# Dostenlinus/Aiyagari-HARK

Hardware: AMD Instinct MI355X
Metric: GE solves/sec (Table II sweep); agent-periods/sec; % HBM roofline (higher is better)
Workload: dtype f64

## Files before the change

aiyagari_hark_amd/csrc/egm_common.h:

```cpp
#pragma once

#include "common.h"

namespace aiy {

constexpr int kEgmBlock = 256;
constexpr int kTile = 64;
constexpr int kEgmWaves = kEgmBlock / kWave;
constexpr int kSub = 32;
constexpr int kFlag = 3 * kSub;
constexpr int kSlots = 3 * kSub + 4;
constexpr int kWin = 2 * kWave;

constexpr int kHintBack = 8;


template <bool AGENT>
__device__ __forceinline__ double ld_f64(const double* p) {
  if constexpr (AGENT) return load_f64_agent(p);
  else return *p;
}

__device__ __forceinline__ double uniform_f64(double x) {
  const unsigned long long u = (unsigned long long)__double_as_longlong(x);
// ... 94 lines not shown

__device__ __forceinline__ double interp_row_global(const double* __restrict__ xr, const double* __restrict__ yr,
                                                    int n, double q, int& lb) {
  lb = lower_bound(xr, 0, n, q);
  const int i = lb < 1 ? 1 : lb;
  return lerp_at(xr, yr, i, q, xr[0]);
}

__device__ __forceinline__ double interp_row_global_agent(const double* __restrict__ xr,
                                                          const double* __restrict__ yr, int n, double q, int& lb) {
  int lo = 0, hi = n;
  while (lo < hi) {
    const int mid = lo + ((hi - lo) >> 1);
    if (load_f64_agent(&xr[mid]) < q) lo = mid + 1; else hi = mid;
  }
  lb = lo;
  const int i = lb < 1 ? 1 : lb;
  const double xl = load_f64_agent(&xr[i - 1]), xh = load_f64_agent(&xr[i]);
  const double yl = load_f64_agent(&yr[i - 1]), yh = load_f64_agent(&yr[i]);
  const double alpha = (q - xl) / (xh - xl);
  const double v = (1.0 - alpha) * yl + alpha * yh;
  return (q < load_f64_agent(&xr[0])) ? __builtin_nan("") : v;
}

template <int PK>
__device__ __forceinline__ double marg_u(double c, double gam) {
  if constexpr (PK == 1) return 1.0 / c;
  else if constexpr (PK == 3) return 1.0 / ((c * c) * c);
  else if constexpr (PK == 5) {
    const double c2 = c * c;
    return 1.0 / ((c2 * c2) * c);
  } else return pow(c, -gam);
}
template <int PK>
__device__ __forceinline__ double inv_marg(double E, double gam) {
  if constexpr (PK == 1) return 1.0 / E;
  else if constexpr (PK == 3) return rcbrt(E);
  else if constexpr (PK == 5) {
    if (!(E > 1e-30 && E < 1e30)) return pow(E, -0.2);
    double y = (double)powf((float)E, -0.2f);
#pragma unroll
    for (int it = 0; it < 2; ++it) {
      const double y2 = y * y;
      const double e = 1.0 - E * ((y2 * y2) * y);
      y = y + y * (e * 0.2);
    }
    return y;
  } else return pow(E, -1.0 / gam);
}

}
```

aiyagari_hark_amd/csrc/ge_resident.hip:

```cpp
#include "common.h"
#include "egm_common.h"
#include "ge_search.h"
#include "hist_bicg.h"
#include "hist_cluster.h"
#include "internal.h"

#include <algorithm>
#include <cmath>

namespace aiy {

constexpr int kGeTHMax = 1024;
constexpr int kGeWavesMax = kGeTHMax / kWave;
constexpr int kGeMaxTiles = 16;
constexpr int kGeBufs = 5;
constexpr int kGeAaM = 3;
constexpr int kGeAaHist = kGeAaM + 2;
#ifdef AIY_DIAG_NO_FUSEA
constexpr bool kGeFuseA = false;
#else
constexpr bool kGeFuseA = true;
#endif
#ifndef AIY_FUSEA_KC2
#define AIY_FUSEA_KC2 0
#endif
constexpr bool kGeFuseAKc2 = AIY_FUSEA_KC2 != 0;
template <int NW>
constexpr size_t ge_egm_lds() { return (size_t)NW * (8 * kTile + 4 * kWin) * sizeof(double); }

struct GeCalDev {
  double alpha, delta, disc, r_lo, r_hi;
};

struct GeState;
struct GeRun {
  int n_cal, S, n_a, G, nj, cap, n_work;
  const double* a_grid;
  const double* P;
  const double* lab;
  const double* beta;
  const double* crra;
  const GeCalDev* cal;
  int method;
  double r_tol, egm_tol, hist_tol;
  int max_steps, max_cyc, max_hist;
  int warm_hist, warm_egm, secant, loose, extrap;
  int extrap_period;
  int aa_period;
  double* aah;
  int logsec;
  int pull;
  double loose_hist;
  double* qb;
  int* ainv;
  double* tab;
  double* mass;
  double* pmass;
  double* pg;
  int* lo;
  double* wlo;
  double* slab;
  int* span;
  unsigned* ctr;
  unsigned long long* gran;
  const int* cal_ids;
  GeState* saved;
  const int* resume;
  unsigned* done_ctr;
  int stop_at;
  int* out_done;
  unsigned* err;
  double* out_r;
  double* out_K;
  double* out_Ks;
  int* out_steps;
  int* out_cyc;
  int* out_its;
  int* out_status;
  double* out_prof;
  double* out_evlog;
};
constexpr int kGeProf = 8;
constexpr int kGeEvLog = 32;
constexpr int kGeEvRec = 6;
// ... 8 lines not shown
  long long cyc_sum, its_sum;
  unsigned long long t_egm, t_lot, t_hist, t_k, t0, t_ev0;
  unsigned nc_prev[2];
  unsigned nbc;
};

template <int TH>
__device__ __forceinline__ bool ge_reduce(unsigned long long* gran, int G, int w, unsigned& ne, const double* vals,
                                          int nv, unsigned kmax, double (*s_part)[kGeWavesMax], double* s_res,
                                          int* s_flag, unsigned* err) {
  asm volatile("s_waitcnt vmcnt(0)" ::: "memory");
  return hc_reduce<TH>(gran, G, w, ne, vals, nv, kmax, s_part, s_res, s_flag, err, [] {});
}

template <int SMAX, int NW, typename Sink, typename Begin, typename End>
__device__ __forceinline__ void ge_rows_pass(int S, int n_a, int j0, int j1, const double* __restrict__ a_grid,
                                             const double* __restrict__ src_m, const double* __restrict__ src_c,
                                             double R, const double* s_Wl, int* s_hint, double* lds_win,
                                             Sink&& sink, Begin&& begin, End&& end) {
  const int tid = threadIdx.x, lane = tid & (kWave - 1);
  const int wv = __builtin_amdgcn_readfirstlane(tid / kWave);
  const int n = n_a, n1 = n_a + 1;
  const int ntile = (j1 - j0 + kTile - 1) / kTile;
  double* X = lds_win + (size_t)wv * 4 * kWin;
  double* Y = X + kWin;
  double* XB = X + 2 * kWin;
  double* YB = X + 3 * kWin;
#pragma unroll 1
  for (int tile = wv; tile < ntile; tile += NW) {
    const int jr = j0 + tile * kTile + lane;
    const int j = jr < j1 ? jr : j1 - 1;
    const double a = a_grid[j];
    int* hint = s_hint + tile * SMAX;
    begin(tile, j);
    auto fetch = [&](int r, RowWin& wn) {
      const int rr = r < S ? r : S - 1;
      load_win<true>(src_m + (size_t)rr * n1, src_c + (size_t)rr * n1, n, win_base(hint[rr], n1), lane, wn);
    };
    unsigned redo = 0u;
    auto step_unit = [&](int u, const RowWin& wa, const RowWin& wb) {
      const int ra = 2 * u, rb = 2 * u + 1;
      if (ra >= S) return;
      const bool has_b = rb < S;
      const int rbb = has_b ? rb : ra;
      const bool na = __any(stage_win(wa, n, X, Y, lane));
      const bool nb = __any(stage_win(wb, n, XB, YB, lane));
      __builtin_amdgcn_fence(__ATOMIC_RELEASE, "wavefront");
      __builtin_amdgcn_wave_barrier();
      __builtin_amdgcn_fence(__ATOMIC_ACQUIRE, "wavefront");
      const double qa = R * a + s_Wl[ra];
      const double qb = R * a + s_Wl[rbb];
      int lba, lbb;
      bool oka, okb;
      const double fa = search_win(wa.base, na, n, qa, X, Y, lba, oka);
      const double fb = search_win(wb.base, nb, n, qb, XB, YB, lbb, okb);
      hint[ra] = __builtin_amdgcn_readfirstlane(lba);
      if (has_b) hint[rb] = __builtin_amdgcn_readfirstlane(lbb);
      if (__any(!oka)) redo |= 1u << ra;
      else sink(tile, jr, j, ra, qa, fa);
      if (has_b) {
        if (__any(!okb)) redo |= 1u << rb;
        else sink(tile, jr, j, rb, qb, fb);
      }
    };
    RowWin a0, b0, a1, b1;
    fetch(0, a0);
    fetch(1, b0);
#pragma unroll 1
    for (int u = 0; 2 * u < S; u += 2) {
      fetch(2 * u + 2, a1);
      fetch(2 * u + 3, b1);
      step_unit(u, a0, b0);
      fetch(2 * u + 4, a0);
      fetch(2 * u + 5, b0);
      step_unit(u + 1, a1, b1);
    }
#pragma unroll 1
    while (redo != 0u) {
      const int s = __builtin_ctz(redo);
      redo &= redo - 1u;
      const double q = R * a + s_Wl[s];
      int lb;
      const double f = interp_row_global_agent(src_m + (size_t)s * n1, src_c + (size_t)s * n1, n, q, lb);
      hint[s] = __builtin_amdgcn_readfirstlane(lb);
      sink(tile, jr, j, s, q, f);
    }
    end(tile, j, a);
  }
}

template <int SMAX, int SC, int PK, int NW>
__device__ __forceinline__ double ge_egm_cycle(int S, int n_a, int j0, int j1, const double* __restrict__ a_grid,
                                               const double* src_m, const double* src_c, double* dst_m,
                                               double* dst_c, bool track, double R, double beta, double gam,
                                               const double* s_Wl, const double* s_Pe, int* s_hint,
                                               double* lds_v, double* lds_win, double* ring) {
  const int tid = threadIdx.x, lane = tid & (kWave - 1);
  const int wv = __builtin_amdgcn_readfirstlane(tid / kWave);
  const int n1 = n_a + 1;
  double* Vw = lds_v + (size_t)wv * SMAX * kTile;
  const int ntile = (j1 - j0 + kTile - 1) / kTile;
  double dmax = 0.0;
  if (src_m == nullptr) {
#pragma unroll 1
    for (int tile = wv; tile < ntile; tile += NW) {
      const int jr = j0 + tile * kTile + lane;
      const int j = jr < j1 ? jr : j1 - 1;
      const double a = a_grid[j];
      for (int sp = 0; sp < S; ++sp) {
        const double c = (R * a + s_Wl[sp]) * 1.0;
        Vw[sp * kTile + lane] = R * marg_u<PK>(c, gam);
      }
      for (int s = 0; s < S; ++s) {
        double sum;
        if constexpr (SC > 0) sum = pairwise_dot<SC>(Vw + lane, s_Pe + s * SC);
        else sum = np_pairwise_sum<SMAX>(S, [&](int t) { return Vw[t * kTile + lane] * uniform_f64(s_Pe[s * S + t]); });
        const double c = inv_marg<PK>(beta * sum, gam);
        store_f64_agent(&dst_m[(size_t)s * n1 + j + 1], a + c);
        store_f64_agent(&dst_c[(size_t)s * n1 + j + 1], c);
        if (ring) store_f64_agent(&ring[(size_t)s * n_a + j], c);
        if (j == 0) {
          store_f64_agent(&dst_m[(size_t)s * n1], kBorrowNode);
          store_f64_agent(&dst_c[(size_t)s * n1], kBorrowNode);
        }
      }
    }
    return 0.0;
  }
  constexpr int NP = SC > 0 ? SC : SMAX;
  double pmv[NP], pcv[NP];
  auto begin = [&](int, int j) {
#pragma unroll
    for (int s = 0; s < NP; ++s) {
      pmv[s] = 0.0;
      pcv[s] = 0.0;
      if (track && s < S) {
        pmv[s] = load_f64_agent(&src_m[(size_t)s * n1 + j + 1]);
        pcv[s] = load_f64_agent(&src_c[(size_t)s * n1 + j + 1]);
      }
    }
  };
  auto end = [&](int, int j, double a) {
#pragma unroll
    for (int s = 0; s < NP; ++s) {
      if (s < S) {
        __builtin_amdgcn_sched_barrier(0);
        double sum;
        if constexpr (SC > 0) sum = pairwise_dot<SC>(Vw + lane, s_Pe + s * SC);
        else sum = np_pairwise_sum<SMAX>(S, [&](int t) { return Vw[t * kTile + lane] * uniform_f64(s_Pe[s * S + t]); });
        const double E = beta * sum;
        const double c = inv_marg<PK>(E, gam);
        const double m = a + c;
        store_f64_agent(&dst_m[(size_t)s * n1 + j + 1], m);
        store_f64_agent(&dst_c[(size_t)s * n1 + j + 1], c);
        if (ring) store_f64_agent(&ring[(size_t)s * n_a + j], c);
        if (track) dmax = nan_max(dmax, nan_max(fabs(m - pmv[s]), fabs(c - pcv[s])));
        if (j == 0) {
          store_f64_agent(&dst_m[(size_t)s * n1], kBorrowNode);
          store_f64_agent(&dst_c[(size_t)s * n1], kBorrowNode);
        }
      }
    }
  };
  ge_rows_pass<SMAX, NW>(S, n_a, j0, j1, a_grid, src_m, src_c, R, s_Wl, s_hint, lds_win,
                     [&](int, int, int, int sp, double, double f) {
                       Vw[sp * kTile + lane] = R * marg_u<PK>(f, gam);
                     },
                     begin, end);
  return dmax;
}

constexpr int kGeSmax = 8;
extern __shared__ double ge_dyn[];
__shared__ double ge_s_part[kHcRed][kGeWavesMax];
__shared__ double ge_s_res[kHcRed];
__shared__ int ge_s_flag;
__shared__ double ge_s_Pe[kGeSmax * kGeSmax];
__shared__ double ge_s_Wl[kGeSmax];
__shared__ int ge_s_hint[kGeMaxTiles * kGeSmax];
__shared__ unsigned ge_s_nc;
__shared__ GeState ge_st;

template <int SMAX, int SC, int PK, int NW>
__device__ __forceinline__ double ge_egm_cycle_fn(int S, int n_a, int j0, int j1, const double* a_grid,
                                               const double* src_m, const double* src_c, double* dst_m,
                                               double* dst_c, bool track, double R, double beta, double gam,
                                               double* ring) {
  return ge_egm_cycle<SMAX, SC, PK, NW>(S, n_a, j0, j1, a_grid, src_m, src_c, dst_m, dst_c, track, R, beta, gam,
                                        ge_s_Wl, ge_s_Pe, ge_s_hint, ge_dyn, ge_dyn + (size_t)NW * SMAX * kTile, ring);
}

template <int SMAX, int NW>
__device__ __forceinline__ void ge_lottery_fn(int S, int n_a, int j0, int j1, const double* a_grid, const double* fm,
                                           const double* fc, double R, bool have_prev, int* LO, double* WL,
                                           bool write_through) {
  ge_rows_pass<SMAX, NW>(S, n_a, j0, j1, a_grid, fm, fc, R, ge_s_Wl, ge_s_hint, ge_dyn + (size_t)NW * SMAX * kTile,
                     [&](int, int jr, int, int s, double q, double c) {
                       if (jr >= j1) return;
                       const double ap = q - c;
                       const size_t o = (size_t)s * n_a + jr;
                       int d = -1;
                       if (have_prev) {
                         const int h = LO[o];
                         if (h >= 0 && h < n_a - 1 && a_grid[h] <= ap && ap < a_grid[h + 1]) d = h;
                       }
                       if (d < 0) {
                         int lo = 0, hi = n_a;
                         while (lo < hi) {
                           const int mid = lo + ((hi - lo) >> 1);
                           if (a_grid[mid] <= ap) lo = mid + 1; else hi = mid;
                         }
                         d = lo - 1;
                       }
                       d = d < 0 ? 0 : (d > n_a - 2 ? n_a - 2 : d);
                       double wl = (a_grid[d + 1] - ap) / (a_grid[d + 1] - a_grid[d]);
                       wl = wl < 0.0 ? 0.0 : (wl > 1.0 ? 1.0 : wl);
                       if (write_through) {
                         __hip_atomic_store(to_global(&LO[o]), d, __ATOMIC_RELAXED, __HIP_MEMORY_SCOPE_AGENT);
                         store_f64_agent(&WL[o], wl);
                       } else {
                         LO[o] = d;
                         WL[o] = wl;
                       }
                     },
                     [](int, int) {}, [](int, int, double) {});
}

struct GeCtx {
  double* tab;
  double* X;
  double* PX;
  int* LO;
  double* WL;
  unsigned* ctr;
  unsigned long long* cw;
  unsigned long long* gran;
  const double* a_grid;
  double beta, gam;
  size_t tab_sz;
  int j0, j1, w, G, S, n_a, cal, lc;
  __device__ __forceinline__ double* tabm(int b) const { return tab + (size_t)b * 2 * tab_sz; }
  __device__ __forceinline__ double* tabc(int b) const { return tab + (size_t)b * 2 * tab_sz + tab_sz; }
};

__device__ __forceinline__ GeEvalOpts ge_eval_opts(const GeRun& g) {
  return {g.method, g.loose, g.logsec, g.warm_egm, g.warm_hist, g.secant, g.r_tol, g.egm_tol, g.hist_tol, g.loose_hist};
}

__device__ __forceinline__ bool ge_barrier(const GeCtx& cx, unsigned& nb, unsigned* err) {
  asm volatile("s_waitcnt vmcnt(0)" ::: "memory");
  ++nb;
  return hc_barrier(err, cx.ctr, (unsigned)cx.G * nb, &ge_s_flag);
}

__device__ __forceinline__ bool ge_vote(const GeCtx& cx, unsigned* err, unsigned flag, unsigned& dlt) {
  GeState& st = ge_st;
  const int tid = threadIdx.x;
  if (tid == 0) ++st.nbc;
  asm volatile("s_waitcnt vmcnt(0)" ::: "memory");
  __syncthreads();
  const unsigned k = st.nbc, par = k & 1u;
  if (!hc_barrier_count(err, &cx.cw[par], (unsigned)cx.G * ((k + par) / 2), flag, &ge_s_nc, &ge_s_flag))
    return false;
  if (tid == 0) {
    dlt = ge_s_nc - st.nc_prev[par];
    st.nc_prev[par] = ge_s_nc;
  }
  return true;
}

template <int TH>
__device__ __forceinline__ void ge_secant_tables(const GeCtx& cx, int b_cur, int b_prev, int b_init, double theta) {
  const int tid = threadIdx.x, n1 = cx.n_a + 1;
  for (int s = 0; s < cx.S; ++s) {
    for (int k = cx.j0 + tid; k < cx.j1; k += TH) {
      const size_t o = (size_t)s * n1 + k + 1;
      const double cm = load_f64_agent(&cx.tabm(b_cur)[o]), pm = load_f64_agent(&cx.tabm(b_prev)[o]);
      const double cc = load_f64_agent(&cx.tabc(b_cur)[o]), pc = load_f64_agent(&cx.tabc(b_prev)[o]);
      store_f64_agent(&cx.tabm(b_init)[o], theta == 0.0 ? cm : cm + theta * (cm - pm));
      store_f64_agent(&cx.tabc(b_init)[o], theta == 0.0 ? cc : cc + theta * (cc - pc));
    }
    if (cx.j0 == 0 && tid == 0) {
      store_f64_agent(&cx.tabm(b_init)[(size_t)s * n1], kBorrowNode);
      store_f64_agent(&cx.tabc(b_init)[(size_t)s * n1], kBorrowNode);
    }
  }
}

template <int SMAX, int SC, int NW>
__device__ __forceinline__ double ge_egm_dispatch(const GeCtx& cx, int pk, const double* sm, const double* sc, double* dm,
                                                  double* dc, bool track, double R, double* ring) {
  if (pk == 1)
    return ge_egm_cycle_fn<SMAX, SC, 1, NW>(cx.S, cx.n_a, cx.j0, cx.j1, cx.a_grid, sm, sc, dm, dc, track, R, cx.beta,
                                            cx.gam, ring);
  if (pk == 3)
    return ge_egm_cycle_fn<SMAX, SC, 3, NW>(cx.S, cx.n_a, cx.j0, cx.j1, cx.a_grid, sm, sc, dm, dc, track, R, cx.beta,
                                            cx.gam, ring);
  if (pk == 5)
    return ge_egm_cycle_fn<SMAX, SC, 5, NW>(cx.S, cx.n_a, cx.j0, cx.j1, cx.a_grid, sm, sc, dm, dc, track, R, cx.beta,
                                            cx.gam, ring);
  return ge_egm_cycle_fn<SMAX, SC, 0, NW>(cx.S, cx.n_a, cx.j0, cx.j1, cx.a_grid, sm, sc, dm, dc, track, R, cx.beta,
                                          cx.gam, ring);
}

template <int TH>
__device__ __forceinline__ bool ge_extrapolate(const GeCtx& cx, unsigned& nb, unsigned* err, int b_dst, int b_src,
                                               double dclu, int n) {
  GeState& st = ge_st;
  const int tid = threadIdx.x, n1 = cx.n_a + 1;
  if (tid == 0) {
    st.fext = egm_extrap_factor(dclu, st.dist, st.ev.etol, n, st.lam_prev);
    if (st.fext != 0.0) st.moved = 1;
  }
  __syncthreads();
  const double f = st.fext;
  if (f != 0.0) {
    double* cm = cx.tabm(b_dst);
    double* cc = cx.tabc(b_dst);
    const double* pm = cx.tabm(b_src);
    const double* pc = cx.tabc(b_src);
    for (int s = 0; s < cx.S; ++s)
      for (int k = cx.j0 + tid; k < cx.j1; k += TH) {
        const size_t o = (size_t)s * n1 + k + 1;
        const double x = load_f64_agent(&cm[o]), y = load_f64_agent(&cc[o]);
        store_f64_agent(&cm[o], x + f * (x - load_f64_agent(&pm[o])));
        store_f64_agent(&cc[o], y + f * (y - load_f64_agent(&pc[o])));
      }
    if (!ge_barrier(cx, nb, err)) return false;
  }
  return true;
}

__device__ __forceinline__ double* ge_ring(const GeCtx& cx, const GeRun& g, int c) {
  return g.aah + ((size_t)cx.cal * kGeAaHist + (size_t)(c % kGeAaHist)) * cx.S * cx.n_a;
}

template <int TH>
__device__ __forceinline__ bool ge_anderson(const GeCtx& cx, unsigned& nb, unsigned& ne, const GeRun& g, int n,
                                            int b_dst) {
  static_assert(kGeAaM == 3 && kGeAaHist == 5, "the mixing is written for m = 3");
  const int tid = threadIdx.x, n1 = cx.n_a + 1;
  const double* W0 = ge_ring(cx, g, n - 4);
  const double* W1 = ge_ring(cx, g, n - 3);
  const double* W2 = ge_ring(cx, g, n - 2);
  const double* W3 = ge_ring(cx, g, n - 1);
  const double* W4 = ge_ring(cx, g, n);
  double gp[9];
  for (int q = 0; q < 9; ++q) gp[q] = 0.0;
  for (int s = 0; s < cx.S; ++s)
    for (int k = cx.j0 + tid; k < cx.j1; k += TH) {
      const size_t o = (size_t)s * cx.n_a + k;
      const double w0 = load_f64_agent(W0 + o), w1 = load_f64_agent(W1 + o), w2 = load_f64_agent(W2 + o);
      const double w3 = load_f64_agent(W3 + o), w4 = load_f64_agent(W4 + o);
      aa_gram_add(w0, w1, w2, w3, w4, gp);
    }
  double gs[9], gam[3];
  if (!ge_reduce<TH>(cx.gran, cx.G, cx.w, ne, gp, 6, 0u, ge_s_part, ge_s_res, &ge_s_flag, g.err)) return false;
  for (int q = 0; q < 6; ++q) gs[q] = ge_s_res[q];
  if (!ge_reduce<TH>(cx.gran, cx.G, cx.w, ne, gp + 6, 3, 0u, ge_s_part, ge_s_res, &ge_s_flag, g.err)) return false;
  for (int q = 0; q < 3; ++q) gs[6 + q] = ge_s_res[q];
  if (aa_solve(gs, gam)) {
    double* dm = cx.tabm(b_dst);
    double* dc = cx.tabc(b_dst);
    for (int s = 0; s < cx.S; ++s)
      for (int k = cx.j0 + tid; k < cx.j1; k += TH) {
        const size_t o = (size_t)s * cx.n_a + k;
        const double w1 = load_f64_agent(W1 + o), w2 = load_f64_agent(W2 + o);
        const double w3 = load_f64_agent(W3 + o), w4 = load_f64_agent(W4 + o);
        const double cn = aa_mix(gam, w1, w2, w3, w4);
        store_f64_agent(&dm[(size_t)s * n1 + k + 1], cx.a_grid[k] + cn);
        store_f64_agent(&dc[(size_t)s * n1 + k + 1], cn);
      }
    if (tid == 0) ge_st.moved = 1;
    if (!ge_barrier(cx, nb, g.err)) return false;
  }
  return true;
}

template <int SMAX, int SC, int TH>
__device__ __forceinline__ int ge_household_solve(const GeCtx& cx, unsigned& nb, unsigned& ne, const GeRun& g, int pk,
                                                  double R, const double* init_m, const double* init_c) {
  constexpr int NW = TH / kWave;
  GeState& st = ge_st;
  const int tid = threadIdx.x;
  int final_buf = -1;
  for (int attempt = 0; attempt < 2; ++attempt) {
    if (!ge_barrier(cx, nb, g.err)) return -1;
    const bool aa = g.aa_period > 0 && attempt == 0;
    const bool ext = st.extrap != 0 && attempt == 0 && !aa;
    if (tid == 0) {
      st.lam_prev = -1.0;
      st.moved = 0;
      st.nan_stop = 0;
    }
    int n = 1;
    const int last_allowed = g.max_cyc + 1;
    bool converged = false;
    while (true) {
      const int b_dst = st.buf[n & 1], b_src = st.buf[(n - 1) & 1];
      const double* sm = n == 1 ? init_m : cx.tabm(b_src);
      const double* sc = n == 1 ? init_c : cx.tabc(b_src);
      const bool track = n >= 2;
      const double dl = ge_egm_dispatch<SMAX, SC, NW>(cx, pk, sm, sc, cx.tabm(b_dst), cx.tabc(b_dst), track, R,
                                                      aa ? ge_ring(cx, g, n) : nullptr);
      const int xp = g.extrap_period;
      const bool want_value = ext && n >= xp - 1 && ((n % xp) == xp - 1 || (n % xp) == 0);
      double dclu = 0.0;
      bool go;
      if (want_value) {
        double v[1] = {dl};
        if (!ge_reduce<TH>(cx.gran, cx.G, cx.w, ne, v, 1, 1u, ge_s_part, ge_s_res, &ge_s_flag, g.err)) return -1;
        dclu = ge_s_res[0];
        go = dclu > st.ev.etol;
        if (tid == 0) st.nan_stop = dclu != dclu;
      } else {
        const double dw = wave_nan_max(dl);
        if ((tid & (kWave - 1)) == 0) ge_s_part[0][tid / kWave] = dw;
        __syncthreads();
        unsigned flag = 0u, dlt = 0u;
        if (tid == 0) {
          double d = ge_s_part[0][0];
          for (int q = 1; q < TH / kWave; ++q) d = nan_max(d, ge_s_part[0][q]);
          flag = (d > st.ev.etol ? 1u : 0u) | (d != d ? (1u << 16) : 0u);
        }
        if (!ge_vote(cx, g.err, flag, dlt)) return -1;
        if (tid == 0) {
          st.stop = (dlt & 0xffffu) == 0u || (dlt >> 16) != 0u;
          st.nan_stop = (dlt >> 16) != 0u;
        }
        __syncthreads();
        go = !st.stop;
      }
      if (track && !go) {
        converged = true;
        break;
      }
      if (n >= last_allowed) break;
      if (want_value && (n % xp) == 0) {
        if (!ge_extrapolate<TH>(cx, nb, g.err, b_dst, b_src, dclu, n)) return -1;
      } else if (want_value) {
        if (tid == 0) st.dist = dclu;
      }
      if (aa && n >= g.aa_period && n >= kGeAaHist + 1 && (n % g.aa_period) == 0) {
        if (!ge_anderson<TH>(cx, nb, ne, g, n, b_dst)) return -1;
      }
      ++n;
    }
    if (tid == 0) {
      st.n = n;
      if (!converged) st.status |= 1;
    }
    __syncthreads();
    final_buf = st.buf[n & 1];
    if (!(st.moved && st.nan_stop)) break;
    if (tid == 0) {
      st.extrap = 0;
      st.status &= ~1;
    }
    __syncthreads();
  }
  return final_buf;
}

template <int TH>
__device__ __forceinline__ void ge_mass_start(const GeCtx& cx, bool fresh, bool warm, bool secant, double theta) {
  const int tid = threadIdx.x;
  if (fresh) {
    const double u0 = 1.0 / ((double)cx.S * cx.n_a);
    for (int s = 0; s < cx.S; ++s)
      for (int k = cx.j0 + tid; k < cx.j1; k += TH) cx.X[(size_t)s * cx.n_a + k] = u0;
  } else if (warm) {
    for (int s = 0; s < cx.S; ++s)
      for (int k = cx.j0 + tid; k < cx.j1; k += TH) {
        const size_t o = (size_t)s * cx.n_a + k;
        const double x = cx.X[o];
        if (secant) cx.X[o] = theta == 0.0 ? x : x + theta * (x - cx.PX[o]);
        cx.PX[o] = x;
      }
  }
}

template <int TH>
__device__ __forceinline__ bool ge_capital(const GeCtx& cx, unsigned& ne, unsigned* err) {
  double part = 0.0;
  for (int k = cx.j0 + (int)threadIdx.x; k < cx.j1; k += TH) {
    double ms = 0.0;
    for (int s = 0; s < cx.S; ++s) ms += cx.X[(size_t)s * cx.n_a + k];
    part += ms * cx.a_grid[k];
  }
  double v[1] = {part};
  return ge_reduce<TH>(cx.gran, cx.G, cx.w, ne, v, 1, 0u, ge_s_part, ge_s_res, &ge_s_flag, err);
}

__device__ __forceinline__ void ge_write_out(const GeCtx& cx, const GeRun& g, const GeCalDev& cd) {
  const GeState& st = ge_st;
  const int cal = cx.cal;
  __hip_atomic_fetch_add(to_global(g.done_ctr), 1u, __ATOMIC_RELAXED, __HIP_MEMORY_SCOPE_AGENT);
  g.out_done[cal] = 1;
  g.out_r[cal] = st.ev.rs.x;
  g.out_K[cal] = ge_prices(st.ev.rs.x, cd.alpha, cd.delta).Kd;
  g.out_Ks[cal] = st.Ks;
  g.out_steps[cal] = st.ev.steps;
  g.out_cyc[cal] = (int)min(st.cyc_sum, 0x7fffffffll);
  g.out_its[cal] = (int)min(st.its_sum, 0x7fffffffll);
  g.out_status[cal] = st.status | (st.ev.rs.done ? 0 : 4);
  double* pf = g.out_prof + (size_t)cal * kGeProf;
  pf[0] = st.t_egm * 0.01;
  pf[1] = st.t_lot * 0.01;
  pf[2] = st.t_hist * 0.01;
  pf[3] = st.t_k * 0.01;
  pf[4] = (__builtin_amdgcn_s_memrealtime() - st.t0) * 0.01;
  pf[5] = (double)st.cyc_sum;
  pf[6] = (double)st.its_sum;
  pf[7] = (double)st.ev.steps;
}

template <int SMAX, int SC, int KC, int TH>
__global__ __launch_bounds__(TH) void ge_cluster_kernel(GeRun g) {
  constexpr int NW = TH / kWave;
  static_assert(SMAX <= kGeSmax, "file-scope LDS sized for kGeSmax states");
  GeState& st = ge_st;

  const int per = gridDim.x >> 3;
  const int u = (blockIdx.x & 7) * per + (blockIdx.x >> 3);
  if (u >= g.n_work) return;
  const int G = g.G, S = g.S, n_a = g.n_a;
  const int tid = threadIdx.x;
  GeCtx cx;
  cx.G = G; cx.S = S; cx.n_a = n_a;
  cx.lc = u / G; cx.w = u - cx.lc * G;
  const int lc = cx.lc, w = cx.w, cal = g.cal_ids[lc];
  cx.cal = cal;
  cx.j0 = w * g.nj; cx.j1 = min(cx.j0 + g.nj, n_a);
  const int j0 = cx.j0, j1 = cx.j1;
  cx.a_grid = g.a_grid + (size_t)cal * n_a;
  cx.beta = g.beta[cal]; cx.gam = g.crra[cal];
  const GeCalDev cd = g.cal[cal];
  cx.tab_sz = (size_t)S * (n_a + 1);
  cx.tab = g.tab + (size_t)cal * kGeBufs * 2 * cx.tab_sz;
  const size_t row0 = (size_t)cal * S * n_a;
  cx.X = g.mass + row0;
  cx.PX = g.pmass + row0;
  cx.LO = g.lo + row0;
  cx.WL = g.wlo + row0;
  cx.ctr = g.ctr + (size_t)lc * kHcCtrStride;
  cx.cw = reinterpret_cast<unsigned long long*>(cx.ctr + 2);
  cx.gran = g.gran + (size_t)lc * 2 * G * kHcRedRec;
  unsigned nb = 0, ne = 0;
  const int pk = cx.gam == 1.0 ? 1 : (cx.gam == 3.0 ? 3 : (cx.gam == 5.0 ? 5 : 0));

  for (int q = tid; q < S * S; q += TH) ge_s_Pe[q] = g.P[(size_t)cal * S * S + q];
  for (int q = tid; q < kGeMaxTiles * SMAX; q += TH) ge_s_hint[q] = -1;
  if (tid == 0) {
    if (g.resume[cal]) {
      st = g.saved[cal];
      st.t0 = __builtin_amdgcn_s_memrealtime() - st.t0;
    } else {
      st.ev.init(ge_eval_opts(g), cd.r_lo, cd.r_hi);
      st.Ks = 0.0;
      st.in_hist = 0;
      st.status = 0;
      st.cyc_sum = st.its_sum = 0;
      for (int b = 0; b < kGeBufs; ++b) st.buf[b] = b;
      st.t_egm = st.t_lot = st.t_hist = st.t_k = 0ull;
      st.t0 = __builtin_amdgcn_s_memrealtime();
    }
    st.opt = ge_eval_opts(g);
    st.nc_prev[0] = st.nc_prev[1] = 0u;
    st.nbc = 0u;
  }
  __syncthreads();

  bool stopped = false;
  while ((!st.ev.rs.done && st.ev.steps < g.max_steps) || st.ev.final_ks) {
    if (g.stop_at > 0 && st.ev.steps > 0 && !st.in_hist) {
      unsigned flag = 0u, dlt = 0u;
      if (tid == 0)
        flag = __hip_atomic_load(to_global(g.done_ctr), __ATOMIC_RELAXED, __HIP_MEMORY_SCOPE_AGENT) >=
                       (unsigned)g.stop_at ? 1u : 0u;
      if (!ge_vote(cx, g.err, flag, dlt)) return;
      if (tid == 0) st.stop = dlt != 0u;
      __syncthreads();
      if (st.stop) {
        stopped = true;
        break;
      }
    }
    unsigned long long tp = __builtin_amdgcn_s_memrealtime();
    if (tid == 0 && !st.in_hist) st.t_ev0 = tp;
    if (!st.in_hist) {
      if (tid == 0) {
        st.ev.plan(st.opt, cd.alpha, cd.delta);
        st.extrap = g.extrap;
        st.moved = 0;
      }
      __syncthreads();
      if (tid < S) ge_s_Wl[tid] = st.ev.wage * g.lab[(size_t)cal * S + tid];
      const double R = st.ev.R, theta = st.ev.theta;
      const bool secant = st.ev.secant != 0, warm = st.ev.warm_egm != 0;
      const int b_cur = st.buf[2], b_prev = st.buf[3], b_init = st.buf[4];
      if (secant) ge_secant_tables<TH>(cx, b_cur, b_prev, b_init, theta);
      tp = __builtin_amdgcn_s_memrealtime();
      const int final_buf = ge_household_solve<SMAX, SC, TH>(
          cx, nb, ne, g, pk, R, secant ? cx.tabm(b_init) : (warm ? cx.tabm(b_cur) : nullptr),
          secant ? cx.tabc(b_init) : (warm ? cx.tabc(b_cur) : nullptr));
      if (final_buf < 0) return;
      if (tid == 0) {
        const unsigned long long tn = __builtin_amdgcn_s_memrealtime();
        st.t_egm += tn - tp;
        st.cyc_sum += st.n;
        const int fb = final_buf;
        const int other = st.buf[0] == fb ? st.buf[1] : st.buf[0];
        const int old_prev = st.buf[3];
        st.buf[3] = st.buf[2];
        st.buf[2] = fb;
        st.buf[0] = other;
        st.buf[1] = old_prev;
      }
      __syncthreads();
      tp = __builtin_amdgcn_s_memrealtime();
      ge_lottery_fn<SMAX, NW>(S, n_a, j0, j1, cx.a_grid, cx.tabm(st.buf[2]), cx.tabc(st.buf[2]), R, st.ev.steps > 0,
                              cx.LO, cx.WL, g.pull != 0);
      ge_mass_start<TH>(cx, st.ev.fresh_mass != 0, warm, secant, theta);
      __syncthreads();
      if (tid == 0) {
        const unsigned long long tn = __builtin_amdgcn_s_memrealtime();
        st.t_lot += tn - tp;
        tp = tn;
      }
    }
    int mv;
    {
      HkArgs hk;
      hk.G = G; hk.S = S; hk.n_a = n_a; hk.cap = g.cap; hk.w = w; hk.j0 = j0; hk.j1 = j1;
      hk.LO = to_global((const int*)cx.LO); hk.WL = to_global((const double*)cx.WL); hk.X = to_global(cx.X);
      hk.Pg = to_global(g.pg + row0); hk.Vg = to_global((double*)nullptr);
      hk.slab_cl = to_global(g.slab + (size_t)lc * G * 2 * g.cap);
      hk.span_cl = to_global(g.span + (size_t)lc * G * SMAX * 4);
      hk.ctr = to_global(cx.ctr); hk.gran = to_global(cx.gran); hk.Pc = to_global(g.P + (size_t)cal * S * S);
      hk.max_iter = g.max_hist; hk.err = to_global(g.err);
      hk.tol = st.ev.htol;
      hk.stop_ctr = to_global((const unsigned*)(g.stop_at > 0 ? g.done_ctr : nullptr));
      hk.stop_at = (unsigned)g.stop_at;
      hk.Qg = to_global(g.qb + row0);
      hk.Ainv = to_global(g.ainv + (size_t)cal * S * (n_a + 1));
      hk.lottery_fresh = true;
      hk.dyn_lds = hk_lds_addr(ge_dyn);
      mv = g.pull ? hk_solve_inlined<SMAX, KC, TH, true, false, SC>(hk, &nb, &ne)
                  : hk_solve_isolated<SMAX, KC, TH, false, (KC == 1 || kGeFuseAKc2) && kGeFuseA, SC>(hk, &nb, &ne);
    }
    if (mv == -1) return;
    if (tid == 0) {
      const unsigned long long tn = __builtin_amdgcn_s_memrealtime();
      st.t_hist += tn - tp;
      tp = tn;
    }
    if (mv <= -2) {
      if (tid == 0) {
        st.its_sum += -mv - 2;
        st.in_hist = 1;
        if (w == 0) __hip_atomic_fetch_add(to_global(g.done_ctr + 1), 1u, __ATOMIC_RELAXED, __HIP_MEMORY_SCOPE_AGENT);
      }
      __syncthreads();
      stopped = true;
      break;
    }
    if (tid == 0) st.in_hist = 0;
    if (!ge_capital<TH>(cx, ne, g.err)) return;
    const bool fin = st.ev.final_ks != 0;
    if (tid == 0) {
      const double Ks = ge_s_res[0];
      if (w == 0 && st.ev.steps < kGeEvLog && !fin) {
        double* ev = g.out_evlog + ((size_t)cal * kGeEvLog + st.ev.steps) * kGeEvRec;
        ev[0] = st.ev.rs.x;
        ev[1] = (Ks - st.ev.Kd) / st.ev.Kd;
        ev[2] = (double)st.n;
        ev[3] = (double)mv;
        ev[4] = (double)st.ev.loose;
        ev[5] = (double)(__builtin_amdgcn_s_memrealtime() - st.t_ev0) * 0.01;
      }
      st.its_sum += mv;
      if (mv >= g.max_hist) st.status |= 2;
    }
    if (fin) {
      if (tid == 0) st.Ks = ge_s_res[0];
      __syncthreads();
      break;
    }
    if (tid == 0) {
      st.ev.accept(ge_s_res[0]);
      st.Ks = ge_s_res[0];
      st.t_k += __builtin_amdgcn_s_memrealtime() - tp;
    }
    __syncthreads();
  }
  if (stopped) {
    if (w == 0 && tid == 0) {
      st.t0 = __builtin_amdgcn_s_memrealtime() - st.t0;
      g.saved[cal] = st;
      g.out_done[cal] = 0;
    }
    return;
  }
  if (w == 0 && tid == 0) ge_write_out(cx, g, cd);
}

struct GePlan {
  int G = 0, nj = 0, kc = 0, smax = 0, sc = 0, cap = 0, blocks = 0, th = 0;
  size_t lds = 0;
  const void* fn = nullptr;
};

template <int SMAX, int SC, int KC, int TH>
static const void* ge_fn() {
  return reinterpret_cast<const void*>(ge_cluster_kernel<SMAX, SC, KC, TH>);
}

static bool ge_make_plan(aiy_handle* h, int n_cal, int S, int n_a, GePlan& p) {
  if (S < 1 || S > kGeSmax || n_a < 2 || n_cal < 1) return false;
  int cus = 0;
  if (hipDeviceGetAttribute(&cus, hipDeviceAttributeMultiprocessorCount, h->device) != hipSuccess || cus < 1) return false;
  if (h->cu_limit > 0) cus = std::min(cus, h->cu_limit);
  const int g_min = (n_a + 2 * 512 - 1) / (2 * 512);
  if (g_min > kHcMaxG || g_min > cus) return false;
  const int g_cap = h->hist_cluster_cap > 0 ? h->hist_cluster_cap : 32;
  int G = std::max(g_min, std::min(std::min(g_cap, kHcMaxG), cus / n_cal));
  G = std::min(G, n_a);
  p.nj = (n_a + G - 1) / G;
  p.G = (n_a + p.nj - 1) / p.nj;
  if (p.G > kHcMaxG) return false;
  if (p.nj > kGeMaxTiles * kTile) return false;
  if ((long long)p.G * n_cal > cus) return false;
  p.th = 512;
  const int th = p.th;
  p.kc = p.nj <= th ? 1 : 2;
  p.smax = S == 7 ? 7 : 8;
  p.sc = S == 7 ? 7 : 0;
  if (p.sc == 7) p.fn = p.kc == 1 ? ge_fn<7, 7, 1, 512>() : ge_fn<7, 7, 2, 512>();
  else p.fn = p.kc == 1 ? ge_fn<8, 0, 1, 512>() : ge_fn<8, 0, 2, 512>();
  hipFuncAttributes fa;
  if (hipFuncGetAttributes(&fa, p.fn) != hipSuccess) return false;
  int lds_dev = 0;
  if (hipDeviceGetAttribute(&lds_dev, hipDeviceAttributeMaxSharedMemoryPerMultiprocessor, h->device) != hipSuccess)
    return false;
  const size_t lds_total = std::min<size_t>(kHcLdsTotal, (size_t)lds_dev);
  const size_t stat = fa.sharedSizeBytes;
  if (stat + 4096 >= lds_total) return false;
  p.lds = (lds_total - stat - 1024) / 256 * 256;
  const size_t vbytes = (size_t)p.kc * p.smax * th * sizeof(double);
  const size_t egm_lds = ge_egm_lds<8>();
  if (p.lds < egm_lds || p.lds <= vbytes + 4096) return false;
  p.cap = (int)((p.lds - vbytes) / sizeof(double));
  p.blocks = (p.G * n_cal + 7) / 8 * 8;
  return true;
}

struct GeScratch {
  size_t tab, mass, pmass, pg, qb, ainv, lo, wlo, slab, span, ctr, gran, ids, saved, resume, done, err, cal, outd, outi, prof,
      evlog, aah, bytes;
};
static GeScratch ge_scratch_layout(int n_cal, int S, int n_a, int cus, int cap_max) {
  GeScratch L;
  size_t o = 0;
  auto take = [&](size_t bytes) { const size_t at = o; o += (bytes + 255) / 256 * 256; return at; };
  const size_t pts = (size_t)n_cal * S * n_a;
  L.tab = take((size_t)n_cal * kGeBufs * 2 * S * (n_a + 1) * sizeof(double));
  L.mass = take(pts * 8); L.pmass = take(pts * 8); L.pg = take(pts * 8); L.qb = take(pts * 8);
  L.ainv = take((size_t)n_cal * S * (n_a + 1) * sizeof(int));
  L.lo = take(pts * 4); L.wlo = take(pts * 8);
  L.slab = take((size_t)cus * 2 * cap_max * sizeof(double));
  L.span = take((size_t)cus * 8 * 4 * sizeof(int));
  L.ctr = take((size_t)n_cal * kHcCtrStride * sizeof(unsigned));
// ... 31 lines not shown
    h->ge_cap = 0;
    AIY_HIP(h, hipMalloc(&h->d_ge, L.bytes));
    h->ge_cap = L.bytes;
  }
  char* base = static_cast<char*>(h->d_ge);
  std::vector<GeCalDev> cals(n_cal);
  for (int c = 0; c < n_cal; ++c) {
    cals[c].alpha = M->alpha[c];
    cals[c].delta = M->delta[c];
    cals[c].disc = M->disc[c];
    cals[c].r_lo = o->r_lo ? o->r_lo[c] : GeEval::default_lo(M->delta[c]);
    cals[c].r_hi = o->r_hi ? o->r_hi[c] : GeEval::default_hi(M->disc[c]);
  }
  GeRun g;
  g.n_cal = n_cal; g.S = S; g.n_a = n_a;
  g.a_grid = M->a_grid; g.P = M->P; g.lab = M->lab; g.beta = M->beta; g.crra = M->crra;
  g.cal = reinterpret_cast<const GeCalDev*>(base + L.cal);
  g.method = o->method; g.r_tol = o->r_tol; g.egm_tol = o->egm_tol; g.hist_tol = o->hist_tol;
  g.max_steps = o->max_steps;
  g.max_cyc = o->max_egm_cycles > 0 ? o->max_egm_cycles : 5000;
  g.max_hist = o->max_hist_iter > 0 ? o->max_hist_iter : 200000;
  g.warm_hist = o->warm_hist != 0; g.warm_egm = o->warm_egm != 0;
  g.secant = o->secant_start != 0; g.loose = o->loose_bracket != 0; g.extrap = o->egm_extrapolate != 0;
  g.extrap_period = h->ge_extrap_period;
  g.aa_period = o->egm_extrapolate != 0 ? h->ge_anderson : 0;
  g.aah = reinterpret_cast<double*>(base + L.aah);
  g.logsec = h->ge_logsec;
  g.tab = reinterpret_cast<double*>(base + L.tab);
  g.mass = reinterpret_cast<double*>(base + L.mass);
  g.pmass = reinterpret_cast<double*>(base + L.pmass);
  g.pg = reinterpret_cast<double*>(base + L.pg);
  g.qb = reinterpret_cast<double*>(base + L.qb);
  g.ainv = reinterpret_cast<int*>(base + L.ainv);
  g.pull = h->hist_pull;
  g.loose_hist = std::pow(10.0, -(double)h->ge_loose_hist);
  g.lo = reinterpret_cast<int*>(base + L.lo);
  g.wlo = reinterpret_cast<double*>(base + L.wlo);
  g.slab = reinterpret_cast<double*>(base + L.slab);
  g.span = reinterpret_cast<int*>(base + L.span);
  g.ctr = reinterpret_cast<unsigned*>(base + L.ctr);
  g.gran = reinterpret_cast<unsigned long long*>(base + L.gran);
  int* d_ids = reinterpret_cast<int*>(base + L.ids);
  int* d_resume = reinterpret_cast<int*>(base + L.resume);
  g.cal_ids = d_ids;
  g.saved = reinterpret_cast<GeState*>(base + L.saved);
  g.resume = d_resume;
  g.out_done = reinterpret_cast<int*>(base + L.done);
  g.err = reinterpret_cast<unsigned*>(base + L.err);
  g.done_ctr = g.err + 1;
  double* outd = reinterpret_cast<double*>(base + L.outd);
  int* outi = reinterpret_cast<int*>(base + L.outi);
  g.out_r = outd; g.out_K = outd + n_cal; g.out_Ks = outd + 2 * n_cal;
  g.out_steps = outi; g.out_cyc = outi + n_cal; g.out_its = outi + 2 * n_cal; g.out_status = outi + 3 * n_cal;
  g.out_prof = reinterpret_cast<double*>(base + L.prof);
  g.out_evlog = reinterpret_cast<double*>(base + L.evlog);
  AIY_HIP(h, hipMemsetAsync(g.out_evlog, 0, (size_t)n_cal * kGeEvLog * kGeEvRec * sizeof(double), st));
  AIY_HIP(h, hipMemcpyAsync(base + L.cal, cals.data(), sizeof(GeCalDev) * n_cal, hipMemcpyHostToDevice, st));
  AIY_HIP(h, hipMemsetAsync(d_resume, 0, (size_t)n_cal * sizeof(int), st));
  AIY_HIP(h, hipMemsetAsync(g.out_done, 0, (size_t)n_cal * sizeof(int), st));
  for (hipEvent_t& e : h->ge_ev)
    if (!e) AIY_HIP(h, hipEventCreate(&e));
  std::vector<int> active(n_cal), done(n_cal, 0), resume(n_cal, 0);
  for (int c = 0; c < n_cal; ++c) active[c] = c;
  h->ge_rounds = 0;
  h->ge_mid_stops = 0;
  while (!active.empty()) {
    const int n = (int)active.size();
// ... 139 lines not shown
```

Baseline: 594.1.

## Isolate household solve into noinline per-CRRA function and template kernel on pull

Moves the household EGM solve into a noinline function specialised on the CRRA exponent, with uniform (scalar) arguments, so that the four inlined EGM variants no longer inflate the register pressure of the main GE kernel. The pull histogram mode becomes a template parameter, replacing a runtime branch. The change also moves the cold pow path out of line, loads begin-row values unconditionally after the first fetches to overlap latency, and writes the Anderson ring only on cycles that need it. The cost is call overhead, argument marshalling and twice as many kernel instantiations.

```diff
diff --git a/aiyagari_hark_amd/csrc/egm_common.h b/aiyagari_hark_amd/csrc/egm_common.h
--- a/aiyagari_hark_amd/csrc/egm_common.h
+++ b/aiyagari_hark_amd/csrc/egm_common.h
@@ -150,12 +150,13 @@
     return 1.0 / ((c2 * c2) * c);
   } else return pow(c, -gam);
 }
+__device__ __noinline__ inline double inv_marg5_cold(double E) { return pow(E, -0.2); }
 template <int PK>
 __device__ __forceinline__ double inv_marg(double E, double gam) {
   if constexpr (PK == 1) return 1.0 / E;
   else if constexpr (PK == 3) return rcbrt(E);
   else if constexpr (PK == 5) {
-    if (!(E > 1e-30 && E < 1e30)) return pow(E, -0.2);
+    if (!(E > 1e-30 && E < 1e30)) return inv_marg5_cold(E);
     double y = (double)powf((float)E, -0.2f);
 #pragma unroll
     for (int it = 0; it < 2; ++it) {
diff --git a/aiyagari_hark_amd/csrc/ge_resident.hip b/aiyagari_hark_amd/csrc/ge_resident.hip
--- a/aiyagari_hark_amd/csrc/ge_resident.hip
+++ b/aiyagari_hark_amd/csrc/ge_resident.hip
@@ -49,7 +49,6 @@
   int aa_period;
   double* aah;
   int logsec;
-  int pull;
   double loose_hist;
   double* qb;
   int* ainv;
@@ -124,7 +123,6 @@
     const int j = jr < j1 ? jr : j1 - 1;
     const double a = a_grid[j];
     int* hint = s_hint + tile * SMAX;
-    begin(tile, j);
     auto fetch = [&](int r, RowWin& wn) {
       const int rr = r < S ? r : S - 1;
       load_win<true>(src_m + (size_t)rr * n1, src_c + (size_t)rr * n1, n, win_base(hint[rr], n1), lane, wn);
@@ -158,6 +156,7 @@
     RowWin a0, b0, a1, b1;
     fetch(0, a0);
     fetch(1, b0);
+    begin(tile, j);
 #pragma unroll 1
     for (int u = 0; 2 * u < S; u += 2) {
       fetch(2 * u + 2, a1);
@@ -224,12 +223,9 @@
   auto begin = [&](int, int j) {
 #pragma unroll
     for (int s = 0; s < NP; ++s) {
-      pmv[s] = 0.0;
-      pcv[s] = 0.0;
-      if (track && s < S) {
-        pmv[s] = load_f64_agent(&src_m[(size_t)s * n1 + j + 1]);
-        pcv[s] = load_f64_agent(&src_c[(size_t)s * n1 + j + 1]);
-      }
+      const int rr = s < S ? s : S - 1;
+      pmv[s] = load_f64_agent(&src_m[(size_t)rr * n1 + j + 1]);
+      pcv[s] = load_f64_agent(&src_c[(size_t)rr * n1 + j + 1]);
     }
   };
   auto end = [&](int, int j, double a) {
@@ -277,9 +273,9 @@
 __device__ __forceinline__ double ge_egm_cycle_fn(int S, int n_a, int j0, int j1, const double* a_grid,
                                                const double* src_m, const double* src_c, double* dst_m,
                                                double* dst_c, bool track, double R, double beta, double gam,
-                                               double* ring) {
+                                               double* dyn, double* ring) {
   return ge_egm_cycle<SMAX, SC, PK, NW>(S, n_a, j0, j1, a_grid, src_m, src_c, dst_m, dst_c, track, R, beta, gam,
-                                        ge_s_Wl, ge_s_Pe, ge_s_hint, ge_dyn, ge_dyn + (size_t)NW * SMAX * kTile, ring);
+                                        ge_s_Wl, ge_s_Pe, ge_s_hint, dyn, dyn + (size_t)NW * SMAX * kTile, ring);
 }
 
 template <int SMAX, int NW>
@@ -328,6 +324,8 @@
   unsigned long long* cw;
   unsigned long long* gran;
   const double* a_grid;
+  double* aah;
+  unsigned* err;
   double beta, gam;
   size_t tab_sz;
   int j0, j1, w, G, S, n_a, cal, lc;
@@ -377,22 +375,6 @@
       store_f64_agent(&cx.tabc(b_init)[(size_t)s * n1], kBorrowNode);
     }
   }
-}
-
-template <int SMAX, int SC, int NW>
-__device__ __forceinline__ double ge_egm_dispatch(const GeCtx& cx, int pk, const double* sm, const double* sc, double* dm,
-                                                  double* dc, bool track, double R, double* ring) {
-  if (pk == 1)
-    return ge_egm_cycle_fn<SMAX, SC, 1, NW>(cx.S, cx.n_a, cx.j0, cx.j1, cx.a_grid, sm, sc, dm, dc, track, R, cx.beta,
-                                            cx.gam, ring);
-  if (pk == 3)
-    return ge_egm_cycle_fn<SMAX, SC, 3, NW>(cx.S, cx.n_a, cx.j0, cx.j1, cx.a_grid, sm, sc, dm, dc, track, R, cx.beta,
-                                            cx.gam, ring);
-  if (pk == 5)
-    return ge_egm_cycle_fn<SMAX, SC, 5, NW>(cx.S, cx.n_a, cx.j0, cx.j1, cx.a_grid, sm, sc, dm, dc, track, R, cx.beta,
-                                            cx.gam, ring);
-  return ge_egm_cycle_fn<SMAX, SC, 0, NW>(cx.S, cx.n_a, cx.j0, cx.j1, cx.a_grid, sm, sc, dm, dc, track, R, cx.beta,
-                                          cx.gam, ring);
 }
 
 template <int TH>
@@ -423,20 +405,19 @@
   return true;
 }
 
-__device__ __forceinline__ double* ge_ring(const GeCtx& cx, const GeRun& g, int c) {
-  return g.aah + ((size_t)cx.cal * kGeAaHist + (size_t)(c % kGeAaHist)) * cx.S * cx.n_a;
+__device__ __forceinline__ double* ge_ring(const GeCtx& cx, int c) {
+  return cx.aah + (size_t)(c % kGeAaHist) * cx.S * cx.n_a;
 }
 
 template <int TH>
-__device__ __forceinline__ bool ge_anderson(const GeCtx& cx, unsigned& nb, unsigned& ne, const GeRun& g, int n,
-                                            int b_dst) {
+__device__ __forceinline__ bool ge_anderson(const GeCtx& cx, unsigned& nb, unsigned& ne, int n, int b_dst) {
   static_assert(kGeAaM == 3 && kGeAaHist == 5, "the mixing is written for m = 3");
   const int tid = threadIdx.x, n1 = cx.n_a + 1;
-  const double* W0 = ge_ring(cx, g, n - 4);
-  const double* W1 = ge_ring(cx, g, n - 3);
-  const double* W2 = ge_ring(cx, g, n - 2);
-  const double* W3 = ge_ring(cx, g, n - 1);
-  const double* W4 = ge_ring(cx, g, n);
+  const double* W0 = ge_ring(cx, n - 4);
+  const double* W1 = ge_ring(cx, n - 3);
+  const double* W2 = ge_ring(cx, n - 2);
+  const double* W3 = ge_ring(cx, n - 1);
+  const double* W4 = ge_ring(cx, n);
   double gp[9];
   for (int q = 0; q < 9; ++q) gp[q] = 0.0;
   for (int s = 0; s < cx.S; ++s)
@@ -447,9 +428,9 @@
       aa_gram_add(w0, w1, w2, w3, w4, gp);
     }
   double gs[9], gam[3];
-  if (!ge_reduce<TH>(cx.gran, cx.G, cx.w, ne, gp, 6, 0u, ge_s_part, ge_s_res, &ge_s_flag, g.err)) return false;
+  if (!ge_reduce<TH>(cx.gran, cx.G, cx.w, ne, gp, 6, 0u, ge_s_part, ge_s_res, &ge_s_flag, cx.err)) return false;
   for (int q = 0; q < 6; ++q) gs[q] = ge_s_res[q];
-  if (!ge_reduce<TH>(cx.gran, cx.G, cx.w, ne, gp + 6, 3, 0u, ge_s_part, ge_s_res, &ge_s_flag, g.err)) return false;
+  if (!ge_reduce<TH>(cx.gran, cx.G, cx.w, ne, gp + 6, 3, 0u, ge_s_part, ge_s_res, &ge_s_flag, cx.err)) return false;
   for (int q = 0; q < 3; ++q) gs[6 + q] = ge_s_res[q];
   if (aa_solve(gs, gam)) {
     double* dm = cx.tabm(b_dst);
@@ -464,20 +445,30 @@
         store_f64_agent(&dc[(size_t)s * n1 + k + 1], cn);
       }
     if (tid == 0) ge_st.moved = 1;
-    if (!ge_barrier(cx, nb, g.err)) return false;
+    if (!ge_barrier(cx, nb, cx.err)) return false;
   }
   return true;
 }
 
-template <int SMAX, int SC, int TH>
-__device__ __forceinline__ int ge_household_solve(const GeCtx& cx, unsigned& nb, unsigned& ne, const GeRun& g, int pk,
-                                                  double R, const double* init_m, const double* init_c) {
+struct GeHhOpt {
+  int max_cyc, aa_period, extrap_period;
+};
+
+__device__ __forceinline__ bool ge_ring_wanted(int n, int p) {
+  const int ph = n % p;
+  const int mix = ph == 0 ? n : n + (p - ph);
+  return (ph == 0 || ph > p - kGeAaHist) && mix >= kGeAaHist + 1;
+}
+
+template <int SMAX, int SC, int PK, int TH>
+__device__ __forceinline__ int ge_household_solve(const GeCtx& cx, unsigned& nb, unsigned& ne, const GeHhOpt& g,
+                                                  double R, const double* init_m, const double* init_c, double* dyn) {
   constexpr int NW = TH / kWave;
   GeState& st = ge_st;
   const int tid = threadIdx.x;
   int final_buf = -1;
   for (int attempt = 0; attempt < 2; ++attempt) {
-    if (!ge_barrier(cx, nb, g.err)) return -1;
+    if (!ge_barrier(cx, nb, cx.err)) return -1;
     const bool aa = g.aa_period > 0 && attempt == 0;
     const bool ext = st.extrap != 0 && attempt == 0 && !aa;
     if (tid == 0) {
@@ -493,15 +484,16 @@
       const double* sm = n == 1 ? init_m : cx.tabm(b_src);
       const double* sc = n == 1 ? init_c : cx.tabc(b_src);
       const bool track = n >= 2;
-      const double dl = ge_egm_dispatch<SMAX, SC, NW>(cx, pk, sm, sc, cx.tabm(b_dst), cx.tabc(b_dst), track, R,
-                                                      aa ? ge_ring(cx, g, n) : nullptr);
+      double* ring = aa && ge_ring_wanted(n, g.aa_period) ? ge_ring(cx, n) : nullptr;
+      const double dl = ge_egm_cycle_fn<SMAX, SC, PK, NW>(cx.S, cx.n_a, cx.j0, cx.j1, cx.a_grid, sm, sc, cx.tabm(b_dst),
+                                                          cx.tabc(b_dst), track, R, cx.beta, cx.gam, dyn, ring);
       const int xp = g.extrap_period;
       const bool want_value = ext && n >= xp - 1 && ((n % xp) == xp - 1 || (n % xp) == 0);
       double dclu = 0.0;
       bool go;
       if (want_value) {
         double v[1] = {dl};
-        if (!ge_reduce<TH>(cx.gran, cx.G, cx.w, ne, v, 1, 1u, ge_s_part, ge_s_res, &ge_s_flag, g.err)) return -1;
+        if (!ge_reduce<TH>(cx.gran, cx.G, cx.w, ne, v, 1, 1u, ge_s_part, ge_s_res, &ge_s_flag, cx.err)) return -1;
         dclu = ge_s_res[0];
         go = dclu > st.ev.etol;
         if (tid == 0) st.nan_stop = dclu != dclu;
@@ -515,7 +507,7 @@
           for (int q = 1; q < TH / kWave; ++q) d = nan_max(d, ge_s_part[0][q]);
           flag = (d > st.ev.etol ? 1u : 0u) | (d != d ? (1u << 16) : 0u);
         }
-        if (!ge_vote(cx, g.err, flag, dlt)) return -1;
+        if (!ge_vote(cx, cx.err, flag, dlt)) return -1;
         if (tid == 0) {
           st.stop = (dlt & 0xffffu) == 0u || (dlt >> 16) != 0u;
           st.nan_stop = (dlt >> 16) != 0u;
@@ -529,12 +521,12 @@
       }
       if (n >= last_allowed) break;
       if (want_value && (n % xp) == 0) {
-        if (!ge_extrapolate<TH>(cx, nb, g.err, b_dst, b_src, dclu, n)) return -1;
+        if (!ge_extrapolate<TH>(cx, nb, cx.err, b_dst, b_src, dclu, n)) return -1;
       } else if (want_value) {
         if (tid == 0) st.dist = dclu;
       }
       if (aa && n >= g.aa_period && n >= kGeAaHist + 1 && (n % g.aa_period) == 0) {
-        if (!ge_anderson<TH>(cx, nb, ne, g, n, b_dst)) return -1;
+        if (!ge_anderson<TH>(cx, nb, ne, n, b_dst)) return -1;
       }
       ++n;
     }
@@ -552,6 +544,44 @@
     __syncthreads();
   }
   return final_buf;
+}
+
+struct GeHhArgs {
+  gptr<double> tab, aah;
+  gptr<unsigned> ctr, err;
+  gptr<unsigned long long> gran;
+  gptr<const double> a_grid, init_m, init_c;
+  double beta, gam, R;
+  int j0, j1, w, G, S, n_a;
+  GeHhOpt opt;
+  unsigned dyn_lds;
+};
+template <int SMAX, int SC, int PK, int TH>
+__device__ __noinline__ int ge_household_isolated(GeHhArgs a, unsigned* nb_io, unsigned* ne_io) {
+  double* dyn = (double*)(lptr<double>)(size_t)(unsigned)hk_uni((int)a.dyn_lds);
+  GeCtx cx;
+  cx.tab = (double*)hk_uni(a.tab);
+  cx.aah = (double*)hk_uni(a.aah);
+  cx.ctr = (unsigned*)hk_uni(a.ctr);
+  cx.cw = reinterpret_cast<unsigned long long*>(cx.ctr + 2);
+  cx.err = (unsigned*)hk_uni(a.err);
+  cx.gran = (unsigned long long*)hk_uni(a.gran);
+  cx.a_grid = (const double*)hk_uni(a.a_grid);
+  cx.X = cx.PX = cx.WL = nullptr;
+  cx.LO = nullptr;
+  cx.beta = hk_uni(a.beta); cx.gam = hk_uni(a.gam);
+  cx.j0 = hk_uni(a.j0); cx.j1 = hk_uni(a.j1); cx.w = hk_uni(a.w); cx.G = hk_uni(a.G);
+  cx.S = SC > 0 ? SC : hk_uni(a.S);
+  cx.n_a = hk_uni(a.n_a);
+  cx.cal = cx.lc = 0;
+  cx.tab_sz = (size_t)cx.S * (cx.n_a + 1);
+  const GeHhOpt opt = {hk_uni(a.opt.max_cyc), hk_uni(a.opt.aa_period), hk_uni(a.opt.extrap_period)};
+  unsigned nb = *nb_io, ne = *ne_io;
+  const int fb = ge_household_solve<SMAX, SC, PK, TH>(cx, nb, ne, opt, hk_uni(a.R), (const double*)hk_uni(a.init_m),
+                                                     (const double*)hk_uni(a.init_c), dyn);
+  *nb_io = nb;
+  *ne_io = ne;
+  return fb;
 }
 
 template <int TH>
@@ -607,7 +637,7 @@
   pf[7] = (double)st.ev.steps;
 }
 
-template <int SMAX, int SC, int KC, int TH>
+template <int SMAX, int SC, int KC, int TH, bool PULL>
 __global__ __launch_bounds__(TH) void ge_cluster_kernel(GeRun g) {
   constexpr int NW = TH / kWave;
   static_assert(SMAX <= kGeSmax, "file-scope LDS sized for kGeSmax states");
@@ -638,6 +668,8 @@
   cx.ctr = g.ctr + (size_t)lc * kHcCtrStride;
   cx.cw = reinterpret_cast<unsigned long long*>(cx.ctr + 2);
   cx.gran = g.gran + (size_t)lc * 2 * G * kHcRedRec;
+  cx.aah = g.aah + (size_t)cal * kGeAaHist * S * n_a;
+  cx.err = g.err;
   unsigned nb = 0, ne = 0;
   const int pk = cx.gam == 1.0 ? 1 : (cx.gam == 3.0 ? 3 : (cx.gam == 5.0 ? 5 : 0));
 
@@ -693,9 +725,19 @@
       const int b_cur = st.buf[2], b_prev = st.buf[3], b_init = st.buf[4];
       if (secant) ge_secant_tables<TH>(cx, b_cur, b_prev, b_init, theta);
       tp = __builtin_amdgcn_s_memrealtime();
-      const int final_buf = ge_household_solve<SMAX, SC, TH>(
-          cx, nb, ne, g, pk, R, secant ? cx.tabm(b_init) : (warm ? cx.tabm(b_cur) : nullptr),
-          secant ? cx.tabc(b_init) : (warm ? cx.tabc(b_cur) : nullptr));
+      GeHhArgs ha;
+      ha.tab = to_global(cx.tab); ha.aah = to_global(cx.aah); ha.ctr = to_global(cx.ctr); ha.err = to_global(g.err);
+      ha.gran = to_global(cx.gran); ha.a_grid = to_global(cx.a_grid);
+      ha.init_m = to_global((const double*)(secant ? cx.tabm(b_init) : (warm ? cx.tabm(b_cur) : nullptr)));
+      ha.init_c = to_global((const double*)(secant ? cx.tabc(b_init) : (warm ? cx.tabc(b_cur) : nullptr)));
+      ha.beta = cx.beta; ha.gam = cx.gam; ha.R = R;
+      ha.j0 = j0; ha.j1 = j1; ha.w = w; ha.G = G; ha.S = S; ha.n_a = n_a;
+      ha.opt = {g.max_cyc, g.aa_period, g.extrap_period};
+      ha.dyn_lds = hk_lds_addr(ge_dyn);
+      const int final_buf = pk == 1   ? ge_household_isolated<SMAX, SC, 1, TH>(ha, &nb, &ne)
+                            : pk == 3 ? ge_household_isolated<SMAX, SC, 3, TH>(ha, &nb, &ne)
+                            : pk == 5 ? ge_household_isolated<SMAX, SC, 5, TH>(ha, &nb, &ne)
+                                      : ge_household_isolated<SMAX, SC, 0, TH>(ha, &nb, &ne);
       if (final_buf < 0) return;
       if (tid == 0) {
         const unsigned long long tn = __builtin_amdgcn_s_memrealtime();
@@ -712,7 +754,7 @@
       __syncthreads();
       tp = __builtin_amdgcn_s_memrealtime();
       ge_lottery_fn<SMAX, NW>(S, n_a, j0, j1, cx.a_grid, cx.tabm(st.buf[2]), cx.tabc(st.buf[2]), R, st.ev.steps > 0,
-                              cx.LO, cx.WL, g.pull != 0);
+                              cx.LO, cx.WL, PULL);
       ge_mass_start<TH>(cx, st.ev.fresh_mass != 0, warm, secant, theta);
       __syncthreads();
       if (tid == 0) {
@@ -738,8 +780,8 @@
       hk.Ainv = to_global(g.ainv + (size_t)cal * S * (n_a + 1));
       hk.lottery_fresh = true;
       hk.dyn_lds = hk_lds_addr(ge_dyn);
-      mv = g.pull ? hk_solve_inlined<SMAX, KC, TH, true, false, SC>(hk, &nb, &ne)
-                  : hk_solve_isolated<SMAX, KC, TH, false, (KC == 1 || kGeFuseAKc2) && kGeFuseA, SC>(hk, &nb, &ne);
+      if constexpr (PULL) mv = hk_solve_inlined<SMAX, KC, TH, true, false, SC>(hk, &nb, &ne);
+      else mv = hk_solve_isolated<SMAX, KC, TH, false, (KC == 1 || kGeFuseAKc2) && kGeFuseA, SC>(hk, &nb, &ne);
     }
     if (mv == -1) return;
     if (tid == 0) {
@@ -804,8 +846,9 @@
 };
 
 template <int SMAX, int SC, int KC, int TH>
-static const void* ge_fn() {
-  return reinterpret_cast<const void*>(ge_cluster_kernel<SMAX, SC, KC, TH>);
+static const void* ge_fn(bool pull) {
+  return pull ? reinterpret_cast<const void*>(ge_cluster_kernel<SMAX, SC, KC, TH, true>)
+              : reinterpret_cast<const void*>(ge_cluster_kernel<SMAX, SC, KC, TH, false>);
 }
 
 static bool ge_make_plan(aiy_handle* h, int n_cal, int S, int n_a, GePlan& p) {
@@ -828,8 +871,9 @@
   p.kc = p.nj <= th ? 1 : 2;
   p.smax = S == 7 ? 7 : 8;
   p.sc = S == 7 ? 7 : 0;
-  if (p.sc == 7) p.fn = p.kc == 1 ? ge_fn<7, 7, 1, 512>() : ge_fn<7, 7, 2, 512>();
-  else p.fn = p.kc == 1 ? ge_fn<8, 0, 1, 512>() : ge_fn<8, 0, 2, 512>();
+  const bool pull = h->hist_pull != 0;
+  if (p.sc == 7) p.fn = p.kc == 1 ? ge_fn<7, 7, 1, 512>(pull) : ge_fn<7, 7, 2, 512>(pull);
+  else p.fn = p.kc == 1 ? ge_fn<8, 0, 1, 512>(pull) : ge_fn<8, 0, 2, 512>(pull);
   hipFuncAttributes fa;
   if (hipFuncGetAttributes(&fa, p.fn) != hipSuccess) return false;
   int lds_dev = 0;
@@ -927,7 +971,6 @@
   g.pg = reinterpret_cast<double*>(base + L.pg);
   g.qb = reinterpret_cast<double*>(base + L.qb);
   g.ainv = reinterpret_cast<int*>(base + L.ainv);
-  g.pull = h->hist_pull;
   g.loose_hist = std::pow(10.0, -(double)h->ge_loose_hist);
   g.lo = reinterpret_cast<int*>(base + L.lo);
   g.wlo = reinterpret_cast<double*>(base + L.wlo);
```

New measurement: 638.2, median of 6. 7.4% higher.
